# AmigoLab/SynthAnatomy

Measured on AMD Instinct MI355X. Metric: vqvae_train_volumes_per_sec, higher is better.
Workload: dtype bf16; 1 GPU; baseline_vqvae no_levels=4 no_channels=256 embedding_dim=32 num_embeddings=2048, 160x224x160 fp32 volumes, training step = fwd + MSE + bwd + EMA codebook update + Adam; batch_per_gpu=8, global_batch=8, parallelism=dp1

## Files before the change

### include/synthanatomy_hip.h

```cpp
#ifndef SYNTHANATOMY_HIP_H
#define SYNTHANATOMY_HIP_H
#include <stdint.h>

#ifdef __cplusplus
extern "C" {
#endif

#define SA_ABI_VERSION 5
enum { SA_F32 = 0, SA_BF16 = 1, SA_F16 = 2  };
enum { SA_ACT_NONE = 0, SA_ACT_RELU = 1, SA_ACT_LRELU = 2, SA_ACT_GELU = 3 };
enum { SA_MASK_NONE = 0, SA_MASK_POS = 1 , SA_MASK_LRELU = 2 ,
       SA_MASK_GELU = 3  };
enum { SA_EINVAL = -1, SA_EUNSUPPORTED = -2, SA_ENOGPU = -3, SA_ECOMM = -4  };
#define SA_MAX_TAPS 64

typedef struct sa_conv_geom {
    int32_t N, Dm, Hm, Wm;
    int32_t Di, Hi, Wi, Cin;
    int32_t Do, Ho, Wo, Cout;
    int32_t cin_valid, cout_valid;
    int32_t KT[3];
    int32_t in_mult[3], tap_step[3], in_off[3];
    int32_t out_mult[3], out_off[3];
    int32_t Kpad;
// ... 8 lines not shown
    int32_t act;
    int32_t mask_mode;
    int32_t add_before_act;
    int32_t out_dtype, add_dtype, mask_dtype;
    float slope;
    void *out_pre;
    void *out_lp;
} sa_epilogue;

int sa_abi_version(void);
const char *sa_last_error(void);
const char *sa_last_conv_kernel(void);
void sa_kernel_log_begin(void);
int sa_kernel_log_read(char *buf, int cap, int stop);

#define SA_DBG_NO_HALO           (1u << 0)
#define SA_DBG_NO_HALO256_FUSE   (1u << 2)
#define SA_DBG_NO_DMA            (1u << 3)
#define SA_DBG_NO_SMALL_TILES    (1u << 4)
#define SA_DBG_NO_FUSED_DB       (1u << 5)
#define SA_DBG_NO_WGRAD_HALO9    (1u << 6)
#define SA_DBG_IM2COL_DIRECT     (1u << 7)
#define SA_DBG_LOCAL_ATTN_EXACT  (1u << 9)
#define SA_DBG_HALO256_4W        (1u << 13)
#define SA_DBG_RESERVED_14       (1u << 14)
#define SA_DBG_DENSE_NARROW      (1u << 15)
#define SA_DBG_NO_KGROUPS        (1u << 17)
#define SA_DBG_RESERVED_19      (1u << 19)
#define SA_DBG_RESERVED_20      (1u << 20)
#define SA_DBG_NO_CELLS256       (1u << 21)
#define SA_DBG_NO_CLASS_LAUNCH    (1u << 22)
#define SA_DBG_NO_STRIP_TILES     (1u << 23)
#define SA_DBG_GENERIC_EPILOGUE   (1u << 24)
#define SA_DBG_FAVOR_SEQ_ALWAYS (1u << 18)
#define SA_DBG_DETERMINISTIC     (1u << 16)
#define SA_DBG_SCAN_EXACT_SHIFT  10
int sa_bench_mfma_bf16(float *scratch, int blocks, int iters, void *stream);
int sa_bench_mfma_bf16_ex(float *scratch, int blocks, int threads, int iters, int shape, void *stream);
uint32_t sa_get_debug_flags(void);
uint32_t sa_set_debug_flags(uint32_t flags);
int sa_epilogue_recipe(const sa_epilogue *ep, int dtype);

int sa_pack_weights(const float *w, void *wpk, int dtype, int rows, int red, int ntaps, const int32_t *tap_lut_host,
                    int64_t s_row, int64_t s_red, int rows_pad, int red_stride, int Kpad, void *stream);
typedef struct sa_pack_desc {
  const float *w;
  void *wpk;
  int32_t tap_lut[SA_MAX_TAPS];
  int64_t s_row, s_red;
  int32_t dtype, rows, red, ntaps, rows_pad, red_stride, Kpad, reserved;
} sa_pack_desc;
int sa_pack_weights_batch(const sa_pack_desc *table, const int32_t *block_first, int n, int total_blocks, void *stream);

int sa_conv_fprop(const sa_conv_geom *g, int dtype, const void *in, const void *wpk, void *out, const sa_epilogue *ep,
                  void *stream);
int sa_conv_fprop_classes(const sa_conv_geom *geoms, int n, int dtype, const void *in, const void *const *wpks, void *out, const sa_epilogue *ep,
                          void *stream);

int sa_resblock_fprop(const sa_conv_geom *g, int dtype, const void *x, const void *w3pk, const float *bias1, const void *w1pk, void *h_out,
                      void *y_out, const sa_epilogue *ep, void *stream);

int sa_conv_wgrad(const sa_conv_geom *g, int dtype, const void *in, const void *gout, float *dw, float *db, const int32_t *tap_lut_host,
                  int64_t s_row, int64_t s_red, void *workspace, int64_t workspace_bytes, void *stream);
int sa_conv1x1_backward(const sa_conv_geom *g, int dtype, const void *in, const void *gout, float *dw, float *db, int64_t s_row, int64_t s_red,
                        void *workspace, int64_t workspace_bytes, const void *dgrad_wpk, void *dx, void *stream);
int64_t sa_conv_wgrad_workspace_bytes(const sa_conv_geom *g, int dtype);

int sa_colsum(const void *g, int dtype, int64_t M, int C, int cstride, float *db, void *stream);

int sa_vq_assign(const float *rows, const float *codebook, int64_t M, int K, int D, int64_t *idx, float *zq_st, void *zq_lp,
                 float *counts, float *dw, float *sqerr, float *wnorm, void *stream);
int sa_vq_ema_update(float *N, float *embed_avg, float *codebook, const float *counts, const float *dw, int K, int D,
                     float decay, float eps, void *stream);
int sa_vq_restart_donors(const float *rows, int64_t M, int D, int64_t row_base, int64_t Mtot, int R, uint64_t seed, uint64_t step, float *donors,
                         void *stream);
int sa_vq_ema_update_restart(float *N, float *embed_avg, float *codebook, const float *counts, const float *dw, int K, int D, float decay, float eps,
                             int32_t *idle, int patience, const float *donors, int R, int32_t *info, void *stream);
int sa_vq_perplexity(const float *counts, int K, int64_t M, float *out, void *stream);
int sa_vq_backward(const float *rows, const float *codebook, const int64_t *idx, const void *g_zq, int g_dtype,
                   const float *g_loss, float beta, int64_t M, int D, void *dz, int dz_dtype, void *stream);
int sa_vq_embed(const float *codebook, const int64_t *idx, int64_t M, int K, int D, void *out, int out_dtype, void *stream);

int sa_cast_pad(const void *src, int src_dtype, int src_c, void *dst, int dst_dtype, int dst_stride, int64_t rows, void *stream);
int sa_subpixel_pool_fwd(const float *c, float *out, int N, int D, int H, int W, void *stream);
int sa_subpixel_pool_bwd(const float *g, void *dc, int dc_dtype, int N, int D, int H, int W, void *stream);
int sa_mse(const float *a, const float *b, int64_t n, float *loss_sum, float *grad, float gscale, void *stream);
int sa_baur_loss(const float *pred, const float *target, int64_t BC, int D, int H, int W, float gdl_factor, int reduction_sum, float gscale, float *sums3,
                 float *grad, float *ws, void *stream);
int64_t sa_baur_loss_workspace_bytes(int64_t BC, int D, int H, int W);
enum { SA_FOURIER_SPECTRAL = 0, SA_FOURIER_HARTLEY = 1, SA_FOURIER_WAVEGAN = 2 };
int sa_fourier_loss(int kind, const float *xp, const float *xy, int64_t B, int C, int D, int H, int W, int prioritise_hf, float factor, double *sums,
                    float *grad, void *ws, void *stream);
int64_t sa_fourier_loss_workspace_bytes(int64_t B, int C, int D, int H, int W);
int sa_ms_ssim(const float *x, const float *y, int B, int C, int D, int H, int W, const float *win, int win_size, int levels, const float *weights,
               float c1, float c2, float *out_b, float *level_means, void *ws, void *stream);
int64_t sa_ms_ssim_workspace_bytes(int B, int C, int D, int H, int W, int win_size, int levels);
enum { SA_AUG_IDENTITY = 0, SA_AUG_AFFINE = 1, SA_AUG_SIGNED_PERM = 2 };
enum { SA_AUG_GAMMA = 1, SA_AUG_SHIFT = 2, SA_AUG_NOISE = 4, SA_AUG_CLAMP = 8 };
typedef struct sa_augment_params {
// ... 262 lines not shown
```

### synthanatomy_amd/_ffi.py

```python
from __future__ import annotations

import ctypes
import os
from ctypes import POINTER, Structure, c_char_p, c_float, c_int, c_int32, c_int64, c_void_p

import torch

HERE = os.path.dirname(os.path.abspath(__file__))
LIB_PATH = os.environ.get("SA_HIP_LIB") or os.path.join(HERE, "libsynthanatomy_hip.so")

SA_F32, SA_BF16, SA_F16 = 0, 1, 2
ACT_NONE, ACT_RELU, ACT_LRELU, ACT_GELU = 0, 1, 2, 3
MASK_NONE, MASK_POS, MASK_LRELU, MASK_GELU = 0, 1, 2, 3
MAX_TAPS = 64


class ConvGeom(Structure):
    _fields_ = [
        ("N", c_int32), ("Dm", c_int32), ("Hm", c_int32), ("Wm", c_int32),
        ("Di", c_int32), ("Hi", c_int32), ("Wi", c_int32), ("Cin", c_int32),
        ("Do", c_int32), ("Ho", c_int32), ("Wo", c_int32), ("Cout", c_int32),
        ("cin_valid", c_int32), ("cout_valid", c_int32),
        ("KT", c_int32 * 3),
        ("in_mult", c_int32 * 3), ("tap_step", c_int32 * 3), ("in_off", c_int32 * 3),
# ... 67 lines not shown
    "sa_last_error": (c_char_p, []),
    "sa_last_conv_kernel": (c_char_p, []),
    "sa_kernel_log_begin": (None, []),
    "sa_kernel_log_read": (c_int, [ctypes.c_char_p, c_int, c_int]),
    "sa_bench_mfma_bf16": (c_int, [c_void_p, c_int, c_int, c_void_p]),
    "sa_bench_mfma_bf16_ex": (c_int, [c_void_p, c_int, c_int, c_int, c_int, c_void_p]),
    "sa_get_debug_flags": (ctypes.c_uint32, []),
    "sa_set_debug_flags": (ctypes.c_uint32, [ctypes.c_uint32]),
    "sa_epilogue_recipe": (c_int, [POINTER(Epilogue), c_int]),
    "sa_conv1_fwd": (c_int, [c_void_p, c_void_p, c_void_p, c_void_p, c_int, c_int, c_int, c_int, c_int, c_int, c_void_p]),
    "sa_conv1_fwd_f16": (c_int, [c_void_p, c_void_p, c_void_p, c_void_p, c_void_p, c_int, c_int, c_int, c_int, c_int, c_int, c_void_p]),
    "sa_conv1_wgrad": (c_int, [c_void_p, c_void_p, c_void_p, c_void_p, c_int, c_int, c_int, c_int, c_int, c_void_p]),
    "sa_convt1_fused_fwd": (c_int, [c_void_p, c_void_p, c_void_p, c_void_p, c_int, c_int, c_int, c_int, c_void_p]),
    "sa_convt1_backward": (c_int, [c_void_p, c_void_p, c_void_p, c_int, c_void_p, c_void_p, c_void_p, c_int, c_int, c_int, c_int, c_void_p]),
    "sa_favor_features_project_bwd": (c_int, [c_void_p, c_void_p, c_void_p, c_void_p, c_int, c_int, c_void_p, c_int, c_void_p, c_void_p, c_void_p, c_int64, c_int,
                                              c_int, c_int, c_void_p]),
    "sa_favor_project_features": (c_int, [c_void_p, c_int, c_int, c_void_p, c_void_p, c_void_p, c_int64, c_int, c_int, c_int, c_void_p]),
    "sa_favor_project": (c_int, [c_void_p, c_int, c_int, c_void_p, c_void_p, c_void_p, c_int64, c_int, c_int, c_int, c_void_p]),
    "sa_favor_project_bwd": (c_int, [c_void_p, c_void_p, c_void_p, c_void_p, c_int, c_int, c_int64, c_int, c_int, c_int, c_void_p]),
    "sa_favor_generalized_features_fwd": (c_int, [c_void_p, c_void_p, c_int64, c_int, c_int, c_void_p]),
    "sa_favor_generalized_features_bwd": (c_int, [c_void_p, c_void_p, c_void_p, c_int64, c_int, c_int, c_void_p]),
    "sa_favor_generalized_project_features": (c_int, [c_void_p, c_int, c_int, c_void_p, c_void_p, c_int64, c_int, c_int, c_int, c_int, c_int64, c_int64, c_void_p]),
    "sa_favor_generalized_project_bwd": (c_int, [c_void_p, c_void_p, c_void_p, c_void_p, c_int, c_int, c_int64, c_int, c_int, c_int, c_int, c_int64, c_int64,
                                                 c_void_p]),
    "sa_favor_generalized_step": (c_int, [c_void_p, c_int, c_int, c_void_p, c_int, c_int, c_void_p, c_int, c_int, c_void_p, c_int, c_int, c_int, c_int, c_int,
                                          c_void_p, c_void_p, c_void_p, c_void_p, c_void_p, c_int, c_int, c_void_p]),
    "sa_pack_weights_batch": (c_int, [c_void_p, c_void_p, c_int, c_int, c_void_p]),
    "sa_pack_weights": (c_int, [c_void_p, c_void_p, c_int, c_int, c_int, c_int, POINTER(c_int32), c_int64, c_int64, c_int, c_int, c_int, c_void_p]),
    "sa_conv_fprop": (c_int, [POINTER(ConvGeom), c_int, c_void_p, c_void_p, c_void_p, POINTER(Epilogue), c_void_p]),
    "sa_conv_fprop_classes": (c_int, [POINTER(ConvGeom), c_int, c_int, c_void_p, POINTER(c_void_p), c_void_p, POINTER(Epilogue), c_void_p]),
    "sa_resblock_fprop": (c_int, [POINTER(ConvGeom), c_int, c_void_p, c_void_p, c_void_p, c_void_p, c_void_p, c_void_p, POINTER(Epilogue), c_void_p]),
    "sa_conv_wgrad": (c_int, [POINTER(ConvGeom), c_int, c_void_p, c_void_p, c_void_p, c_void_p, POINTER(c_int32), c_int64, c_int64, c_void_p, c_int64, c_void_p]),
    "sa_conv_wgrad_workspace_bytes": (c_int64, [POINTER(ConvGeom), c_int]),
    "sa_conv1x1_backward": (c_int, [POINTER(ConvGeom), c_int, c_void_p, c_void_p, c_void_p, c_void_p, c_int64, c_int64, c_void_p, c_int64, c_void_p, c_void_p,
                                    c_void_p]),
    "sa_colsum": (c_int, [c_void_p, c_int, c_int64, c_int, c_int, c_void_p, c_void_p]),
    "sa_vq_assign": (c_int, [c_void_p, c_void_p, c_int64, c_int, c_int, c_void_p, c_void_p, c_void_p, c_void_p, c_void_p, c_void_p, c_void_p, c_void_p]),
    "sa_vq_ema_update": (c_int, [c_void_p, c_void_p, c_void_p, c_void_p, c_void_p, c_int, c_int, c_float, c_float, c_void_p]),
    "sa_vq_restart_donors": (c_int, [c_void_p, c_int64, c_int, c_int64, c_int64, c_int, ctypes.c_uint64, ctypes.c_uint64, c_void_p, c_void_p]),
    "sa_vq_ema_update_restart": (c_int, [c_void_p, c_void_p, c_void_p, c_void_p, c_void_p, c_int, c_int, c_float, c_float, c_void_p, c_int, c_void_p, c_int,
                                         c_void_p, c_void_p]),
    "sa_vq_perplexity": (c_int,[c_void_p, c_int, c_int64, c_void_p, c_void_p]),
    "sa_vq_backward": (c_int, [c_void_p, c_void_p, c_void_p, c_void_p, c_int, c_void_p, c_float, c_int64, c_int, c_void_p, c_int, c_void_p]),
    "sa_vq_embed": (c_int, [c_void_p, c_void_p, c_int64, c_int, c_int, c_void_p, c_int, c_void_p]),
    "sa_cast_pad": (c_int, [c_void_p, c_int, c_int, c_void_p, c_int, c_int, c_int64, c_void_p]),
    "sa_mse": (c_int, [c_void_p, c_void_p, c_int64, c_void_p, c_void_p, c_float, c_void_p]),
    "sa_mse_det": (c_int, [c_void_p, c_void_p, c_int64, c_void_p, c_void_p, c_float, c_void_p, c_void_p]),
    "sa_baur_loss": (c_int, [c_void_p, c_void_p, c_int64, c_int, c_int, c_int, c_float, c_int, c_float, c_void_p, c_void_p, c_void_p, c_void_p]),
    "sa_baur_loss_workspace_bytes": (c_int64, [c_int64, c_int, c_int, c_int]),
    "sa_fourier_loss": (c_int, [c_int, c_void_p, c_void_p, c_int64, c_int, c_int, c_int, c_int, c_int, c_float, c_void_p, c_void_p, c_void_p, c_void_p]),
    "sa_fourier_loss_workspace_bytes": (c_int64, [c_int64, c_int, c_int, c_int, c_int]),
    "sa_ms_ssim": (c_int, [c_void_p, c_void_p, c_int, c_int, c_int, c_int, c_int, c_void_p, c_int, c_int, c_void_p, c_float, c_float, c_void_p, c_void_p,
                           c_void_p, c_void_p]),
    "sa_ms_ssim_workspace_bytes": (c_int64, [c_int, c_int, c_int, c_int, c_int, c_int, c_int]),
    "sa_augment": (c_int, [c_void_p, c_void_p, c_int, c_int, c_int, c_int, c_int, c_int, c_int, c_void_p, ctypes.c_uint64, c_void_p, c_void_p]),
    "sa_augment_workspace_bytes": (c_int64, [c_int]),
    "sa_volume_ingest": (c_int, [c_void_p, c_int64, c_void_p, c_void_p, c_void_p, c_void_p]),
    "sa_volume_ingest_workspace_bytes": (c_int64, []),
    "sa_volume_egress": (c_int, [c_void_p, c_void_p, c_int64, c_void_p, c_void_p, c_void_p]),
    "sa_volume_egress_workspace_bytes": (c_int64, []),
    "sa_anomaly_map": (c_int, [c_void_p, c_void_p, c_void_p, c_void_p, c_void_p, POINTER(AnomalyParams), c_void_p, c_void_p, c_void_p]),
    "sa_anomaly_map_workspace_bytes": (c_int64, [POINTER(AnomalyParams)]),
    "sa_anomaly_map_ensemble": (c_int, [c_void_p, c_void_p, c_int64, c_void_p, c_int64, c_void_p, c_void_p, POINTER(AnomalyParams), c_int, c_void_p,
                                        c_void_p, c_void_p]),
    "sa_components": (c_int, [c_void_p, c_void_p, c_void_p, POINTER(ComponentsParams), c_void_p, c_void_p, c_void_p]),
    "sa_components_workspace_bytes": (c_int64, [POINTER(ComponentsParams)]),
# ... 183 lines not shown
```

### synthanatomy_amd/csrc/conv_wgrad.hip

```cpp
#include <stdio.h>
#include <stdlib.h>

#include "sa_common.h"

namespace sa {

struct WgradArgs {
    const void* in;
    const void* gout;
    float* dw;
    sa_conv_geom g;
    FastDiv dW, dH, dD, dTw, dThw, dCin;
    int32_t lut[SA_MAX_TAPS];
    int64_t s_row, s_red;
    uint32_t M, ntaps, ktot;
    uint32_t chunks_per_split, nchunks;
    uint32_t nkt, ntiles;
    uint32_t in_bytes, g_bytes;
    float* ws;
    float* db;
    const void* dg_wpk;
    void* dg_out;
    uint32_t HQ, WP, nsteps, steps_per_split, halo;
    FastDiv dWP, dHQ;
};

template <typename T> struct WG;
template <> struct WG<bf16_t> { static constexpr int MK = 64; };
template <> struct WG<float> { static constexpr int MK = 16; };

__device__ __forceinline__ uint32_t roff(uint32_t m, uint32_t c) { return m * 256u + ((((c >> 4) ^ (m & 7u)) << 5) | ((c & 15u) << 1)); }

typedef short v4s_t __attribute__((ext_vector_type(4)));
__device__ __forceinline__ v4s_t lds_tr16(const unsigned char* p) {
    return __builtin_amdgcn_ds_read_tr16_b64_v4i16((__attribute__((address_space(3))) v4s_t*)(p));
}

__device__ __forceinline__ void dma16_hidden(__amdgpu_buffer_rsrc_t rsrc, uint32_t lds_addr, uint32_t voff) {
    asm volatile("s_mov_b32 m0, %0\n\ts_nop 0\n\tbuffer_load_dwordx4 %1, %2, 0 offen lds" : : "s"(lds_addr), "v"(voff), "s"(rsrc) : "memory", "m0");
}
__device__ __forceinline__ void dma_wait() { asm volatile("s_waitcnt vmcnt(0)" ::: "memory"); }
__device__ __forceinline__ uint32_t lds_address(const void* p) { return (uint32_t)(uintptr_t)(__attribute__((address_space(3))) const void*)p; }

template <int ROWS, int NGROUPS>
__device__ __forceinline__ void tile_colsum(const unsigned char* pg, uint32_t tid, float& s0, float& s1) {
    const uint32_t cp = tid & 63u, rg = tid >> 6;
#pragma unroll
    for (int m = 0; m < ROWS / NGROUPS + (ROWS % NGROUPS ? 1 : 0); ++m) {
        const uint32_t row = rg + (uint32_t)m * NGROUPS;
        if (ROWS % NGROUPS == 0 || row < (uint32_t)ROWS) {
            const uint32_t v = *(const uint32_t*)(pg + roff(row, 2u * cp));
            s0 += __uint_as_float(v << 16);
            s1 += __uint_as_float(v & 0xffff0000u);
        }
    }
}
// ... 548 lines not shown
        for (int ks = 0; ks < PHS / 2; ++ks) {
            short8_t xf[4], gf[4];
            const uint32_t xr0 = (uint32_t)(2 * ks) * 18u + tw + trow, xr1 = xr0 + 18u;
#pragma unroll
            for (int i = 0; i < 4; ++i) {
                const v4s_t lo = lds_tr16(px + roff(xr0, wm * 64 + i * 16 + tcol));
                const v4s_t hi = lds_tr16(px + roff(xr1, wm * 64 + i * 16 + tcol));
                xf[i] = __builtin_shufflevector(lo, hi, 0, 1, 2, 3, 4, 5, 6, 7);
            }
#pragma unroll
            for (int j = 0; j < 4; ++j) {
                const v4s_t lo = lds_tr16(pg + roff(ks * 32 + trow, wn * 64 + j * 16 + tcol));
                const v4s_t hi = lds_tr16(pg + roff(ks * 32 + 16 + trow, wn * 64 + j * 16 + tcol));
                gf[j] = __builtin_shufflevector(lo, hi, 0, 1, 2, 3, 4, 5, 6, 7);
            }
#pragma unroll
            for (int i = 0; i < 4; ++i)
#pragma unroll
                for (int j = 0; j < 4; ++j) acc[i][j] = __builtin_amdgcn_mfma_f32_16x16x32_bf16(xf[i], gf[j], acc[i][j], 0, 0, 0);
        }
        __syncthreads();
    }
    if (do_db) colsum_finish<12>((float*)smem, tid, bs0, bs1, a.db, ct * 128u, (uint32_t)g.cout_valid);
    const uint32_t tile = (td * 3u + th) * 3u + tw + a.nkt * ct;
    float* wt = a.ws + ((size_t)split * a.ntiles + tile) * (128 * 128);
#pragma unroll
    for (int i = 0; i < 4; ++i)
#pragma unroll
        for (int j = 0; j < 4; ++j) *(float4_t*)(wt + (wn * 64 + j * 16 + frow) * 128 + wm * 64 + i * 16 + fq * 4) = acc[i][j];
#endif
}

__device__ __forceinline__ uint32_t roff128(uint32_t m, uint32_t c) { return m * 128u + ((((c >> 4) ^ ((m >> 1) & 3u)) << 5) | ((c & 15u) << 1)); }

template <int NW>
__global__ __launch_bounds__(NW * 64) void conv_wgrad_halo9_kernel(const WgradArgs a) {
#if defined(__HIP_DEVICE_COMPILE__)
    constexpr int NJ = 32 / NW;
    constexpr int XP = 23, GP = 32, NP = XP + GP, PPW = (NP + NW - 1) / NW;
    constexpr int XT = XP * 1024, GT = GP * 1024, STAGE = XT + GT;
    extern __shared__ __attribute__((aligned(16))) unsigned char smem[];
    const sa_conv_geom& g = a.g;
    const uint32_t tid = threadIdx.x, lane = tid & 63u;
    const uint32_t wave = __builtin_amdgcn_readfirstlane(tid >> 6);
    const uint32_t fi = wave & 3u, wn = wave >> 2;
    const uint32_t nct = a.ntiles / a.nkt;
    const uint32_t xcd = blockIdx.x & 7u, seq = blockIdx.x >> 3;
    const uint32_t per_split = 6u * nct;
    const uint32_t nsplit = (a.nsteps + a.steps_per_split - 1) / a.steps_per_split;
    const uint32_t spx = (nsplit + 7u) >> 3;
    const uint32_t sl = seq / per_split, rem = seq - sl * per_split;
    const uint32_t split = xcd * spx + sl;
    if (sl >= spx || split >= nsplit) return;
    const uint32_t tdc = rem % 6u, ct = rem / 6u;
    const uint32_t td = tdc >> 1, cih = tdc & 1u;
    const uint32_t step0 = split * a.steps_per_split;
    uint32_t step1 = step0 + a.steps_per_split;
    if (step1 > a.nsteps) step1 = a.nsteps;

    float4_t acc[9][NJ];
#pragma unroll
    for (int t = 0; t < 9; ++t)
#pragma unroll
        for (int j = 0; j < NJ; ++j) acc[t][j] = (float4_t){0.f, 0.f, 0.f, 0.f};

    __amdgpu_buffer_rsrc_t rX = __builtin_amdgcn_make_buffer_rsrc((void*)a.in, 0, (int)a.in_bytes, 0x00020000);
// ... 18 lines not shown
            p_h[i] = (int32_t)(r >> 4);
            p_w[i] = (int32_t)(r & 15u);
            p_off[i] = (uint32_t)((p_h[i] * g.Wo + p_w[i]) * (g.Cout * 2)) + ct * 256u + vec * 16u;
        }
    }
    auto issue = [&](uint32_t step, uint32_t buf) __attribute__((always_inline)) {
        const uint32_t ps = smem_addr + buf * STAGE;
        uint32_t q1 = fdiv(step, a.dWP);
        const uint32_t wp = step - q1 * a.WP;
        uint32_t q2 = fdiv(q1, a.dHQ);
        const uint32_t hq = q1 - q2 * a.HQ;
        const uint32_t n = fdiv(q2, a.dD);
        const uint32_t d = q2 - n * (uint32_t)g.Dm;
        const int32_t h0 = (int32_t)hq * 8, w0 = (int32_t)wp * 16;
        const int32_t id = (int32_t)d + g.in_off[0] + (int32_t)td;
        const bool dok = (uint32_t)id < (uint32_t)g.Di;
        const uint32_t xbase = (uint32_t)((((int32_t)n * g.Di + id) * g.Hi + h0) * g.Wi + w0) * (uint32_t)(g.Cin * 2);
        const uint32_t gbase = (uint32_t)((((int32_t)n * g.Do + (int32_t)d) * g.Ho + h0) * g.Wo + w0) * (uint32_t)(g.Cout * 2);
#pragma unroll
        for (int i = 0; i < PPW; ++i) {
            const uint32_t q = wave + (uint32_t)NW * i;
            if (q >= (uint32_t)NP) break;
            const int32_t hh = h0 + p_h[i], ww = w0 + p_w[i];
            if (q < (uint32_t)XP) {
                const bool ok = dok && (uint32_t)hh < (uint32_t)g.Hi && (uint32_t)ww < (uint32_t)g.Wi;
                dma16_hidden(rX, ps + q * 1024, ok ? xbase + p_off[i] : 0xfffffff0u);
            } else {
                const bool ok = (uint32_t)hh < (uint32_t)g.Ho && (uint32_t)ww < (uint32_t)g.Wo;
                dma16_hidden(rG, ps + XT + (q - (uint32_t)XP) * 1024, ok ? gbase + p_off[i] : 0xfffffff0u);
            }
        }
    };

    issue(step0, 0);
    dma_wait();
    __syncthreads();
    const uint32_t frow = lane & 15u, fq = lane >> 4;
    const uint32_t trow = fq * 4u + (frow >> 2), tcol = (frow & 3u) * 4u;
    const bool do_db = a.db != nullptr && tdc == 0u;
    float bs0 = 0.f, bs1 = 0.f;
    uint32_t xa[9][2];
#pragma unroll
    for (int t = 0; t < 9; ++t) {
        const uint32_t xr0 = (uint32_t)(t / 3) * 18u + (uint32_t)(t % 3) + trow;
        xa[t][0] = roff128(xr0, fi * 16 + tcol);
        xa[t][1] = roff128(xr0 + 18u, fi * 16 + tcol);
    }
    uint32_t ga[NJ];
#pragma unroll
    for (int j = 0; j < NJ; ++j) ga[j] = roff(trow, wn * (16 * NJ) + j * 16 + tcol);
    for (uint32_t st = step0; st < step1; ++st) {
        const uint32_t buf = (st - step0) & 1u;
        if (st + 1 < step1) issue(st + 1, buf ^ 1u);
        const unsigned char* px = smem + buf * STAGE;
        const unsigned char* pg = px + XT;
        if (do_db) tile_colsum<128, NW>(pg, tid, bs0, bs1);
#pragma unroll 1
        for (uint32_t ks = 0; ks < 4; ++ks) {
            short8_t gf[NJ];
            const unsigned char* pgk = pg + ks * 8192u;
            const unsigned char* pxk = px + ks * 4608u;
            const uint32_t kx = (ks & 1u) * 64u;
#pragma unroll
            for (int j = 0; j < NJ; ++j) {
                const v4s_t lo = lds_tr16(pgk + ga[j]);
                const v4s_t hi = lds_tr16(pgk + ga[j] + 4096);
                gf[j] = __builtin_shufflevector(lo, hi, 0, 1, 2, 3, 4, 5, 6, 7);
            }
#pragma unroll
            for (int t = 0; t < 9; ++t) {
                const v4s_t lo = lds_tr16(pxk + (xa[t][0] ^ kx));
                const v4s_t hi = lds_tr16(pxk + (xa[t][1] ^ kx));
                const short8_t xf = __builtin_shufflevector(lo, hi, 0, 1, 2, 3, 4, 5, 6, 7);
#pragma unroll
                for (int j = 0; j < NJ; ++j) acc[t][j] = __builtin_amdgcn_mfma_f32_16x16x32_bf16(xf, gf[j], acc[t][j], 0, 0, 0);
            }
        }
        dma_wait();
        __syncthreads();
    }
    if (do_db) colsum_finish<NW>((float*)smem, tid, bs0, bs1, a.db, ct * 128u, (uint32_t)g.cout_valid);
#pragma unroll
    for (int t = 0; t < 9; ++t) {
        float* wt = a.ws + ((size_t)split * a.ntiles + (td * 9u + t) + a.nkt * ct) * (128 * 128);
#pragma unroll
        for (int j = 0; j < NJ; ++j) *(float4_t*)(wt + (wn * (16 * NJ) + j * 16 + frow) * 128 + cih * 64 + fi * 16 + fq * 4) = acc[t][j];
    }
#endif
}

__global__ __launch_bounds__(256) void wgrad_reduce_kernel(const WgradArgs a, uint32_t splits) {
    const uint32_t e4 = blockIdx.x * blockDim.x + threadIdx.x;
    if (e4 >= a.ntiles * 4096u) return;
    const uint32_t e = e4 * 4u;
    const uint32_t tile = e >> 14, co_l = (e >> 7) & 127u, k_l = e & 127u;
    const uint32_t kt = tile % a.nkt, ct = tile / a.nkt;
    const uint32_t kidx = kt * 128u + k_l, co = ct * 128u + co_l;
    if (kidx >= a.ktot || co >= (uint32_t)a.g.cout_valid) return;
    float4_t s = (float4_t){0.f, 0.f, 0.f, 0.f};
    const float* p = a.ws + e;
    const size_t stride = (size_t)a.ntiles * 16384u;
    uint32_t sp = 0;
    for (; sp + 8 <= splits; sp += 8) {
        float4_t v[8];
#pragma unroll
        for (int u = 0; u < 8; ++u) v[u] = __builtin_nontemporal_load((const float4_t*)(p + (size_t)(sp + u) * stride));
#pragma unroll
        for (int u = 0; u < 8; ++u) s += v[u];
    }
    for (; sp < splits; ++sp) s += *(const float4_t*)(p + (size_t)sp * stride);
#pragma unroll
    for (int r = 0; r < 4; ++r) {
        const uint32_t kk = kidx + r;
        if (kk >= a.ktot) break;
        const uint32_t tap = fdiv(kk, a.dCin);
        const uint32_t c = kk - tap * a.g.Cin;
        if (c >= (uint32_t)a.g.cin_valid) continue;
        a.dw[co * a.s_row + (int64_t)c * a.s_red + a.lut[tap]] += s[r];
    }
}

__global__ __launch_bounds__(1024) void wgrad_reduce_wide_kernel(const WgradArgs a, uint32_t splits) {
// ... 101 lines not shown
    const int64_t M = (int64_t)g->N * g->Dm * g->Hm * g->Wm;
    if (M <= 0 || M >= (1ll << 31)) return SA_EINVAL;
    a.g = *g;
    a.dW = make_fastdiv(g->Wm);
    a.dH = make_fastdiv(g->Hm);
    a.dD = make_fastdiv(g->Dm);
    a.dTw = make_fastdiv(g->KT[2]);
    a.dThw = make_fastdiv(g->KT[1] * g->KT[2]);
    a.dCin = make_fastdiv(g->Cin);
    a.M = (uint32_t)M;
    a.ntaps = ntaps;
    a.ktot = ntaps * g->Cin;
    const int mk = dtype == SA_F32 ? 16 : 64;
    a.nchunks = (uint32_t)((M + mk - 1) / mk);
    a.nkt = (a.ktot + 127) / 128;
    const uint32_t nct = ((uint32_t)g->cout_valid + 127) / 128;
    a.ntiles = a.nkt * nct;
    const int target_rows = g_tunables.wgrad_rows;
    const uint32_t want_cps = (uint32_t)(target_rows / mk) ? (uint32_t)(target_rows / mk) : 1u;
    splits = (a.nchunks + want_cps - 1) / want_cps;
    const uint32_t env_blocks = (uint32_t)g_tunables.wgrad_min_blocks;
    const uint32_t min_blocks = env_blocks ? env_blocks : ((ntaps == 1 && a.nchunks <= 1024u) ? 512u : 1024u);
    const uint32_t min_splits = (min_blocks + a.ntiles - 1) / a.ntiles;
    if (splits < min_splits) splits = min_splits;
    const uint32_t cap = (uint32_t)((2ull << 30) / ((uint64_t)a.ntiles * 65536ull));
    if (splits > cap && cap >= 1) splits = cap;
    const uint32_t min_chunks = dtype == SA_F32 ? 16 : 4;
    uint32_t max_splits = (a.nchunks + min_chunks - 1) / min_chunks;
    if (splits > max_splits) splits = max_splits;
    if (splits < 1) splits = 1;
    a.chunks_per_split = (a.nchunks + splits - 1) / splits;
    splits = (a.nchunks + a.chunks_per_split - 1) / a.chunks_per_split;
    a.halo = 0;
    {
        bool ok = dtype == SA_BF16 && g->Cin == 128 && g->cin_valid == 128 && g->Cout % 128 == 0 && !dbg(SA_DBG_NO_HALO) && !dbg(SA_DBG_NO_DMA);
        for (int d = 0; d < 3 && ok; ++d)
            ok = g->KT[d] == 3 && g->in_mult[d] == 1 && g->tap_step[d] == 1 && g->in_off[d] == -1 && g->out_mult[d] == 1 && g->out_off[d] == 0;
        ok = ok && g->Dm == g->Do && g->Hm == g->Ho && g->Wm == g->Wo && g->Di == g->Do && g->Hi == g->Ho && g->Wi == g->Wo;
        const uint64_t ib = (uint64_t)g->N * g->Di * g->Hi * g->Wi * g->Cin * 2, gb = (uint64_t)g->N * g->Do * g->Ho * g->Wo * g->Cout * 2;
        ok = ok && ib < 0xffffff00ull - (1u << 20) && gb < 0xffffff00ull - (1u << 20);
        if (ok) {
            const bool nine = !dbg(SA_DBG_NO_WGRAD_HALO9);
            const uint32_t phs = nine ? 8u : 4u;
            const uint32_t hq = (uint32_t)(g->Ho + phs - 1) / phs, wp = (uint32_t)(g->Wo + 15) / 16;
            const double eff = (double)g->Ho * g->Wo / ((double)hq * phs * wp * 16);
            const uint64_t nsteps = (uint64_t)g->N * g->Dm * hq * wp;
            if (eff >= 0.8 && nsteps >= 512) {
                a.halo = nine ? 9u : 4u;
                a.HQ = hq;
                a.WP = wp;
                a.nsteps = (uint32_t)nsteps;
                a.dWP = make_fastdiv(wp);
                a.dHQ = make_fastdiv(hq);
                const int want = g_tunables.wgrad_halo_splits ? g_tunables.wgrad_halo_splits : (nine ? 128 : 256);
                uint32_t sp = (uint32_t)want;
                if (sp > a.nsteps / 16) sp = a.nsteps / 16;
                if (sp < 1) sp = 1;
                a.steps_per_split = (a.nsteps + sp - 1) / sp;
                splits = (a.nsteps + a.steps_per_split - 1) / a.steps_per_split;
            }
        }
    }
    return 0;
}
}

extern "C" int64_t sa_conv_wgrad_workspace_bytes(const sa_conv_geom* g, int dtype) {
    using namespace sa;
    if (!g) return SA_EINVAL;
    WgradArgs a;
    uint32_t splits;
    const int rc = plan_wgrad(g, dtype, a, splits);
    if (rc) return rc;
    return (int64_t)splits * a.ntiles * 128 * 128 * 4;
}

extern "C" int sa_colsum(const void* gp, int dtype, int64_t M, int C, int cstride, float* db, void* stream);

static int conv_wgrad_impl(const sa_conv_geom* g, int dtype, const void* in, const void* gout, float* dw, float* db, const int32_t* tap_lut_host,
                           int64_t s_row, int64_t s_red, void* workspace, int64_t workspace_bytes, const void* dg_wpk, void* dg_out, void* stream) {
    using namespace sa;
    if (!g || !in || !gout || !dw) return SA_EINVAL;
    WgradArgs a;
    uint32_t splits;
    const int rc = plan_wgrad(g, dtype, a, splits);
    if (rc) return rc;
    a.in = in;
    a.gout = gout;
    a.dw = dw;
    const int ntaps = a.ntaps;
    for (int t = 0; t < SA_MAX_TAPS; ++t) a.lut[t] = tap_lut_host ? (t < ntaps ? tap_lut_host[t] : 0) : t;
    a.s_row = s_row;
    a.s_red = s_red;
    const int64_t need = (int64_t)splits * a.ntiles * 128 * 128 * 4;
    a.ws = (workspace && workspace_bytes >= need) ? (float*)workspace : nullptr;
    if (workspace && !a.ws) return SA_EINVAL;
    a.db = nullptr;
    const size_t lds = dtype == SA_F32 ? 4 * 8192 : 4 * 16384;
    const uint32_t splits8 = (splits + 7u) & ~7u;
    dim3 grid(a.ntiles * splits8);
    hipStream_t st = (hipStream_t)stream;
    {
        const int sz = dtype == SA_F32 ? 4 : 2;
        const uint64_t ib = (uint64_t)g->N * g->Di * g->Hi * g->Wi * g->Cin * sz, gb = (uint64_t)g->N * g->Do * g->Ho * g->Wo * g->Cout * sz;
        const bool fits = ib < 0xffffff00ull && gb < 0xffffff00ull && !dbg(SA_DBG_NO_DMA);
        a.in_bytes = fits ? (uint32_t)ib : 0u;
        a.g_bytes = fits ? (uint32_t)gb : 0u;
// ... 92 lines not shown
```

### synthanatomy_amd/csrc/elementwise.hip

```cpp
#include "sa_common.h"

#include <cstring>
#include <mutex>
#include <string>

namespace sa {

thread_local hipError_t g_last_error = hipSuccess;
thread_local char g_last_conv_kernel[128] = "";
std::atomic<bool> g_kernel_log_on{false};
static std::mutex g_kernel_log_mu;
static std::string* g_kernel_log = nullptr;
void note_kernel_slow(const char* name) {
    std::lock_guard<std::mutex> lk(g_kernel_log_mu);
    if (!g_kernel_log) g_kernel_log = new std::string();
    std::string key(name);
    if (key.size() > 2 && key.front() == '(' && key.back() == ')') key = key.substr(1, key.size() - 2);
    key.push_back('\n');
    if (g_kernel_log->rfind(key, 0) == 0 || g_kernel_log->find("\n" + key) != std::string::npos) return;
    g_kernel_log->append(key);
}

static uint32_t flags_from_env() {
    auto on = [](const char* n) { return getenv(n) != nullptr; };
    auto num = [](const char* n, int dflt) { const char* e = getenv(n); return e ? atoi(e) : dflt; };
    uint32_t f = 0;
    if (on("SA_NO_HALO")) f |= SA_DBG_NO_HALO;
    if (on("SA_NO_HALO256_FUSE")) f |= SA_DBG_NO_HALO256_FUSE;
    if (on("SA_NO_DMA")) f |= SA_DBG_NO_DMA;
    if (on("SA_NO_SMALL_TILES")) f |= SA_DBG_NO_SMALL_TILES;
    if (on("SA_NO_FUSED_DB")) f |= SA_DBG_NO_FUSED_DB;
    if (getenv("SA_WGRAD_HALO9") && num("SA_WGRAD_HALO9", 1) == 0) f |= SA_DBG_NO_WGRAD_HALO9;
    if (on("SA_IM2COL_DIRECT")) f |= SA_DBG_IM2COL_DIRECT;
    if (on("SA_HALO256_4W")) f |= SA_DBG_HALO256_4W;
    if (on("SA_DENSE_NARROW")) f |= SA_DBG_DENSE_NARROW;
    if (on("SA_DETERMINISTIC")) f |= SA_DBG_DETERMINISTIC;
    if (on("SA_NO_KGROUPS")) f |= SA_DBG_NO_KGROUPS;
    if (on("SA_FAVOR_SEQ_ALWAYS")) f |= SA_DBG_FAVOR_SEQ_ALWAYS;
    if (on("SA_NO_CELLS256")) f |= SA_DBG_NO_CELLS256;
    if (on("SA_NO_CLASS_LAUNCH")) f |= SA_DBG_NO_CLASS_LAUNCH;
    if (on("SA_GENERIC_EPILOGUE")) f |= SA_DBG_GENERIC_EPILOGUE;
    if (num("SA_LOCAL_ATTN_EXACT", 0) == 1) f |= SA_DBG_LOCAL_ATTN_EXACT;
    f |= ((uint32_t)num("SA_SCAN_EXACT", 0) & 7u) << SA_DBG_SCAN_EXACT_SHIFT;
    return f;
}
static Tunables tunables_from_env() {
    auto num = [](const char* n, int dflt) { const char* e = getenv(n); return e ? atoi(e) : dflt; };
    return Tunables{num("SA_WGRAD_ROWS", 10240), num("SA_WGRAD_MIN_BLOCKS", 0), num("SA_WGRAD_HALO_SPLITS", 0), (uint32_t)num("SA_PP_DBG", 0)};
}
std::atomic<uint32_t> g_debug_flags{flags_from_env()};
const Tunables g_tunables = tunables_from_env();

struct PackArgs {
    const float* w;
    void* wpk;
    int32_t lut[SA_MAX_TAPS];
    int64_t s_row, s_red;
    int32_t dtype, rows, red, ntaps, rows_pad, red_stride, Kpad;
};

__global__ void pack_weights_kernel(const PackArgs a) {
    const int64_t total = (int64_t)a.rows_pad * a.Kpad;
    for (int64_t e = (int64_t)blockIdx.x * blockDim.x + threadIdx.x; e < total; e += (int64_t)gridDim.x * blockDim.x) {
        const int r = (int)(e / a.Kpad);
        const int k = (int)(e - (int64_t)r * a.Kpad);
        const int t = k / a.red_stride;
        const int c = k - t * a.red_stride;
        float v = 0.f;
        if (r < a.rows && t < a.ntaps && c < a.red) v = a.w[r * a.s_row + c * a.s_red + a.lut[t]];
        store_from_f32(a.wpk, a.dtype, e, v);
    }
}

__global__ __launch_bounds__(256) void pack_weights_batch_kernel(const sa_pack_desc* __restrict__ table, const int32_t* __restrict__ block_first, int n) {
// ... 411 lines not shown
```

### synthanatomy_amd/debug.py

```python
from __future__ import annotations

import contextlib
import os

LIB_FLAGS = dict(no_halo=1 << 0, no_halo256_fuse=1 << 2, no_dma=1 << 3, no_small_tiles=1 << 4, no_fused_db=1 << 5,
                 no_wgrad_halo9=1 << 6, im2col_direct=1 << 7, local_attn_exact=1 << 9, halo256_4w=1 << 13, dense_narrow=1 << 15, deterministic=1 << 16, no_kgroups=1 << 17, favor_seq_always=1 << 18, no_cells256=1 << 21, no_class_launch=1 << 22, no_strip_tiles=1 << 23, generic_epilogue=1 << 24)
SCAN_EXACT_SHIFT = 10

_HOST_ENV = dict(no_fused_res="SA_NO_FUSED_RES", no_fused_1x1_bwd="SA_NO_FUSED_1X1_BWD", no_fused_qkv="SA_NO_FUSED_QKV", no_fused_favor="SA_NO_FUSED_FAVOR",
                 no_convt1_fused_bwd="SA_NO_CONVT1_FUSED_BWD", no_convt1_fused_fwd="SA_NO_CONVT1_FUSED_FWD", no_side_wgrad="SA_NO_SIDE_WGRAD", no_side_wgrad_vqvae="SA_NO_SIDE_WGRAD_VQVAE",
                 ddp_single_rank="SA_DDP_SINGLE_RANK",
                 no_f16_forward="SA_NO_F16_FORWARD",
                 no_sample_step="SA_NO_SAMPLE_STEP",
                 opt_in_backward="SA_OPT_IN_BACKWARD",
                 share_device="SA_SHARE_DEVICE",
                 no_proj_bf16="SA_NO_PROJ_BF16",
                 keep_ipc_mode="SA_KEEP_IPC_MODE")
_host = {k: os.environ.get(v) is not None for k, v in _HOST_ENV.items()}


def host(name: str) -> bool:
    return _host[name]


def deterministic() -> bool:
    from . import _ffi
    return bool(_ffi.lib().sa_get_debug_flags() & LIB_FLAGS["deterministic"])


def set_deterministic(on: bool = True):
    from . import _ffi
    lib = _ffi.lib()
    f = lib.sa_get_debug_flags()
    lib.sa_set_debug_flags((f | LIB_FLAGS["deterministic"]) if on else (f & ~LIB_FLAGS["deterministic"]))


@contextlib.contextmanager
def override(**kw):
    from . import _ffi
# ... 21 lines not shown
```

Before: 73.33 volumes/s.

## Restructure halo9 wgrad main loop with incremental walk, precomputed masks and staggered DMA

Result: faster. 74.58 volumes/s (median of 6 runs) (+1.7%).

```diff
diff --git a/include/synthanatomy_hip.h b/include/synthanatomy_hip.h
--- a/include/synthanatomy_hip.h
+++ b/include/synthanatomy_hip.h
@@ -64,6 +64,8 @@
 #define SA_DBG_NO_CLASS_LAUNCH    (1u << 22)
 #define SA_DBG_NO_STRIP_TILES     (1u << 23)
 #define SA_DBG_GENERIC_EPILOGUE   (1u << 24)
+#define SA_DBG_WGRAD9_LOCKSTEP    (1u << 25)
+#define SA_DBG_WGRAD9_FORCE       (1u << 26)
 #define SA_DBG_FAVOR_SEQ_ALWAYS (1u << 18)
 #define SA_DBG_DETERMINISTIC     (1u << 16)
 #define SA_DBG_SCAN_EXACT_SHIFT  10
@@ -97,6 +99,7 @@
 int sa_conv1x1_backward(const sa_conv_geom *g, int dtype, const void *in, const void *gout, float *dw, float *db, int64_t s_row, int64_t s_red,
                         void *workspace, int64_t workspace_bytes, const void *dgrad_wpk, void *dx, void *stream);
 int64_t sa_conv_wgrad_workspace_bytes(const sa_conv_geom *g, int dtype);
+int sa_wgrad9_step_walk(uint32_t WP, uint32_t HQ, uint32_t Dm, uint32_t step0, uint32_t count, uint32_t *out);
 
 int sa_colsum(const void *g, int dtype, int64_t M, int C, int cstride, float *db, void *stream);
 
diff --git a/synthanatomy_amd/_ffi.py b/synthanatomy_amd/_ffi.py
--- a/synthanatomy_amd/_ffi.py
+++ b/synthanatomy_amd/_ffi.py
@@ -123,6 +123,7 @@
     "sa_resblock_fprop": (c_int, [POINTER(ConvGeom), c_int, c_void_p, c_void_p, c_void_p, c_void_p, c_void_p, c_void_p, POINTER(Epilogue), c_void_p]),
     "sa_conv_wgrad": (c_int, [POINTER(ConvGeom), c_int, c_void_p, c_void_p, c_void_p, c_void_p, POINTER(c_int32), c_int64, c_int64, c_void_p, c_int64, c_void_p]),
     "sa_conv_wgrad_workspace_bytes": (c_int64, [POINTER(ConvGeom), c_int]),
+    "sa_wgrad9_step_walk": (c_int, [ctypes.c_uint32, ctypes.c_uint32, ctypes.c_uint32, ctypes.c_uint32, ctypes.c_uint32, POINTER(ctypes.c_uint32)]),
     "sa_conv1x1_backward": (c_int, [POINTER(ConvGeom), c_int, c_void_p, c_void_p, c_void_p, c_void_p, c_int64, c_int64, c_void_p, c_int64, c_void_p, c_void_p,
                                     c_void_p]),
     "sa_colsum": (c_int, [c_void_p, c_int, c_int64, c_int, c_int, c_void_p, c_void_p]),
diff --git a/synthanatomy_amd/csrc/conv_wgrad.hip b/synthanatomy_amd/csrc/conv_wgrad.hip
--- a/synthanatomy_amd/csrc/conv_wgrad.hip
+++ b/synthanatomy_amd/csrc/conv_wgrad.hip
@@ -1,5 +1,7 @@
 #include <stdio.h>
 #include <stdlib.h>
+
+#include <type_traits>
 
 #include "sa_common.h"
 
@@ -22,6 +24,7 @@
     const void* dg_wpk;
     void* dg_out;
     uint32_t HQ, WP, nsteps, steps_per_split, halo;
+    uint32_t wg9_lockstep;
     FastDiv dWP, dHQ;
 };
 
@@ -636,6 +639,56 @@
 }
 
 __device__ __forceinline__ uint32_t roff128(uint32_t m, uint32_t c) { return m * 128u + ((((c >> 4) ^ ((m >> 1) & 3u)) << 5) | ((c & 15u) << 1)); }
+
+struct Wgrad9Walk {
+    uint32_t wp, hq, d, n;
+};
+__host__ __device__ inline Wgrad9Walk wgrad9_walk_at(uint32_t step, uint32_t WP, uint32_t HQ, uint32_t Dm) {
+    Wgrad9Walk w;
+    const uint32_t q1 = step / WP, q2 = q1 / HQ;
+    w.wp = step - q1 * WP;
+    w.hq = q1 - q2 * HQ;
+    w.n = q2 / Dm;
+    w.d = q2 - w.n * Dm;
+    return w;
+}
+__host__ __device__ inline void wgrad9_walk_next(Wgrad9Walk& w, uint32_t WP, uint32_t HQ, uint32_t Dm) {
+    if (++w.wp != WP) return;
+    w.wp = 0;
+    if (++w.hq != HQ) return;
+    w.hq = 0;
+    if (++w.d != Dm) return;
+    w.d = 0;
+    ++w.n;
+}
+
+__device__ __forceinline__ v4s_t lds_tr16_at(uint32_t addr) {
+    return __builtin_amdgcn_ds_read_tr16_b64_v4i16((__attribute__((address_space(3))) v4s_t*)(size_t)addr);
+}
+
+#ifdef SA_TIMING
+#define SA_WG9_TROWS 4096
+__device__ unsigned long long g_wg9_timing[SA_WG9_TROWS * 16];
+#define WG9_TNOW(v)                                                                                  \
+    do {                                                                                             \
+        __builtin_amdgcn_sched_barrier(0);                                                           \
+        asm volatile("s_memtime %0\n\ts_waitcnt lgkmcnt(0)" : "=s"(v)::"memory");                     \
+        __builtin_amdgcn_sched_barrier(0);                                                           \
+    } while (0)
+#define WG9_T(slot)                          \
+    do {                                     \
+        unsigned long long t_now_;           \
+        WG9_TNOW(t_now_);                    \
+        wg9_ts[slot] += t_now_ - wg9_tprev;  \
+        wg9_tprev = t_now_;                  \
+    } while (0)
+#else
+#define WG9_T(slot)
+#endif
+
+#ifndef SA_WG9_STAGGER
+#define SA_WG9_STAGGER 1
+#endif
 
 template <int NW>
 __global__ __launch_bounds__(NW * 64) void conv_wgrad_halo9_kernel(const WgradArgs a) {
@@ -720,9 +773,10 @@
         }
     };
 
-    issue(step0, 0);
-    dma_wait();
-    __syncthreads();
+#ifdef SA_TIMING
+    unsigned long long wg9_ts[8] = {0, 0, 0, 0, 0, 0, 0, 0}, wg9_tprev;
+    WG9_TNOW(wg9_tprev);
+#endif
     const uint32_t frow = lane & 15u, fq = lane >> 4;
     const uint32_t trow = fq * 4u + (frow >> 2), tcol = (frow & 3u) * 4u;
     const bool do_db = a.db != nullptr && tdc == 0u;
@@ -737,45 +791,192 @@
     uint32_t ga[NJ];
 #pragma unroll
     for (int j = 0; j < NJ; ++j) ga[j] = roff(trow, wn * (16 * NJ) + j * 16 + tcol);
-    for (uint32_t st = step0; st < step1; ++st) {
-        const uint32_t buf = (st - step0) & 1u;
-        if (st + 1 < step1) issue(st + 1, buf ^ 1u);
-        const unsigned char* px = smem + buf * STAGE;
-        const unsigned char* pg = px + XT;
-        if (do_db) tile_colsum<128, NW>(pg, tid, bs0, bs1);
-#pragma unroll 1
-        for (uint32_t ks = 0; ks < 4; ++ks) {
-            short8_t gf[NJ];
-            const unsigned char* pgk = pg + ks * 8192u;
-            const unsigned char* pxk = px + ks * 4608u;
-            const uint32_t kx = (ks & 1u) * 64u;
-#pragma unroll
-            for (int j = 0; j < NJ; ++j) {
-                const v4s_t lo = lds_tr16(pgk + ga[j]);
-                const v4s_t hi = lds_tr16(pgk + ga[j] + 4096);
-                gf[j] = __builtin_shufflevector(lo, hi, 0, 1, 2, 3, 4, 5, 6, 7);
-            }
-#pragma unroll
-            for (int t = 0; t < 9; ++t) {
-                const v4s_t lo = lds_tr16(pxk + (xa[t][0] ^ kx));
-                const v4s_t hi = lds_tr16(pxk + (xa[t][1] ^ kx));
-                const short8_t xf = __builtin_shufflevector(lo, hi, 0, 1, 2, 3, 4, 5, 6, 7);
-#pragma unroll
-                for (int j = 0; j < NJ; ++j) acc[t][j] = __builtin_amdgcn_mfma_f32_16x16x32_bf16(xf, gf[j], acc[t][j], 0, 0, 0);
-            }
-        }
+    const bool lockstep = NW != 8 || a.wg9_lockstep != 0u || (smem_addr & 127u) != 0u;
+    if (lockstep) {
+        issue(step0, 0);
         dma_wait();
         __syncthreads();
+        WG9_T(6);
+        for (uint32_t st = step0; st < step1; ++st) {
+            const uint32_t buf = (st - step0) & 1u;
+            if (st + 1 < step1) issue(st + 1, buf ^ 1u);
+            WG9_T(0);
+            const unsigned char* px = smem + buf * STAGE;
+            const unsigned char* pg = px + XT;
+            if (do_db) tile_colsum<128, NW>(pg, tid, bs0, bs1);
+            WG9_T(1);
+#pragma unroll 1
+            for (uint32_t ks = 0; ks < 4; ++ks) {
+                short8_t gf[NJ];
+                const unsigned char* pgk = pg + ks * 8192u;
+                const unsigned char* pxk = px + ks * 4608u;
+                const uint32_t kx = (ks & 1u) * 64u;
+#pragma unroll
+                for (int j = 0; j < NJ; ++j) {
+                    const v4s_t lo = lds_tr16(pgk + ga[j]);
+                    const v4s_t hi = lds_tr16(pgk + ga[j] + 4096);
+                    gf[j] = __builtin_shufflevector(lo, hi, 0, 1, 2, 3, 4, 5, 6, 7);
+                }
+#pragma unroll
+                for (int t = 0; t < 9; ++t) {
+                    const v4s_t lo = lds_tr16(pxk + (xa[t][0] ^ kx));
+                    const v4s_t hi = lds_tr16(pxk + (xa[t][1] ^ kx));
+                    const short8_t xf = __builtin_shufflevector(lo, hi, 0, 1, 2, 3, 4, 5, 6, 7);
+                    if (t == 0) WG9_T(2);
+#pragma unroll
+                    for (int j = 0; j < NJ; ++j) acc[t][j] = __builtin_amdgcn_mfma_f32_16x16x32_bf16(xf, gf[j], acc[t][j], 0, 0, 0);
+                }
+                WG9_T(3);
+            }
+            dma_wait();
+            WG9_T(4);
+            __syncthreads();
+            WG9_T(5);
+        }
+    } else {
+        __builtin_assume(wave < (uint32_t)NW);
+        constexpr int NPM = (PPW + 4) / 5;
+        uint32_t pm[NPM];
+#pragma unroll
+        for (int i = 0; i < NPM; ++i) pm[i] = 0u;
+        const int32_t hl = (int32_t)(a.HQ - 1u) * 8, wl = (int32_t)(a.WP - 1u) * 16;
+#pragma unroll
+        for (int i = 0; i < PPW; ++i) {
+            const uint32_t q = wave + (uint32_t)NW * i;
+            uint32_t f;
+            if (q < (uint32_t)XP)
+                f = (p_h[i] < 0 ? 1u : 0u) | (hl + p_h[i] >= g.Hi ? 2u : 0u) | (p_w[i] < 0 ? 4u : 0u) | (wl + p_w[i] >= g.Wi ? 8u : 0u) | (p_h[i] < -1 ? 16u : 0u) | 32u;
+            else
+                f = (hl + p_h[i] >= g.Ho ? 2u : 0u) | (wl + p_w[i] >= g.Wo ? 8u : 0u);
+            pm[i / 5] |= f << (6 * (i % 5));
+        }
+        auto issue2 = [&](const Wgrad9Walk& w, uint32_t buf) __attribute__((always_inline)) {
+            const uint32_t ps = smem_addr + buf * STAGE;
+            const int32_t h0 = (int32_t)w.hq * 8, w0 = (int32_t)w.wp * 16;
+            const int32_t id = (int32_t)w.d + g.in_off[0] + (int32_t)td;
+            const bool dok = (uint32_t)id < (uint32_t)g.Di;
+            const uint32_t xbase = (uint32_t)((((int32_t)w.n * g.Di + id) * g.Hi + h0) * g.Wi + w0) * (uint32_t)(g.Cin * 2);
+            const uint32_t gbase = (uint32_t)((((int32_t)w.n * g.Do + (int32_t)w.d) * g.Ho + h0) * g.Wo + w0) * (uint32_t)(g.Cout * 2);
+            const uint32_t em = (w.hq == 0u ? 1u : 0u) | (w.hq + 1u == a.HQ ? 2u : 0u) | (w.wp == 0u ? 4u : 0u) | (w.wp + 1u == a.WP ? 8u : 0u) | 16u | (dok ? 0u : 32u);
+#pragma unroll
+            for (int i = 0; i < PPW; ++i) {
+                const uint32_t q = wave + (uint32_t)NW * i;
+                if (q >= (uint32_t)NP) break;
+                const bool ok = (pm[i / 5] & (em << (6 * (i % 5)))) == 0u;
+                if (q < (uint32_t)XP) dma16_hidden(rX, ps + q * 1024, ok ? xbase + p_off[i] : 0xfffffff0u);
+                else dma16_hidden(rG, ps + XT + (q - (uint32_t)XP) * 1024, ok ? gbase + p_off[i] : 0xfffffff0u);
+            }
+        };
+        Wgrad9Walk walk;
+        {
+            const uint32_t q1 = fdiv(step0, a.dWP), q2 = fdiv(q1, a.dHQ);
+            walk.wp = step0 - q1 * a.WP;
+            walk.hq = q1 - q2 * a.HQ;
+            walk.n = fdiv(q2, a.dD);
+            walk.d = q2 - walk.n * (uint32_t)g.Dm;
+        }
+        issue2(walk, 0);
+        uint32_t xr[9][2], gr[NJ];
+#pragma unroll
+        for (int t = 0; t < 9; ++t) {
+            xr[t][0] = smem_addr + xa[t][0];
+            xr[t][1] = smem_addr + xa[t][1];
+        }
+#pragma unroll
+        for (int j = 0; j < NJ; ++j) gr[j] = smem_addr + (uint32_t)XT + ga[j];
+        auto kstep = [&](auto ksc) __attribute__((always_inline)) {
+            constexpr uint32_t KS = decltype(ksc)::value;
+            short8_t gf[NJ];
+#pragma unroll
+            for (int j = 0; j < NJ; ++j) {
+                const v4s_t lo = lds_tr16_at(gr[j] + KS * 8192u);
+                const v4s_t hi = lds_tr16_at(gr[j] + KS * 8192u + 4096u);
+                gf[j] = __builtin_shufflevector(lo, hi, 0, 1, 2, 3, 4, 5, 6, 7);
+            }
+#pragma unroll
+            for (int t = 0; t < 9; ++t) {
+                const v4s_t lo = lds_tr16_at((xr[t][0] ^ ((KS & 1u) * 64u)) + KS * 4608u);
+                const v4s_t hi = lds_tr16_at((xr[t][1] ^ ((KS & 1u) * 64u)) + KS * 4608u);
+                const short8_t xf = __builtin_shufflevector(lo, hi, 0, 1, 2, 3, 4, 5, 6, 7);
+                if (t == 0) WG9_T(2);
+#pragma unroll
+                for (int j = 0; j < NJ; ++j) acc[t][j] = __builtin_amdgcn_mfma_f32_16x16x32_bf16(xf, gf[j], acc[t][j], 0, 0, 0);
+            }
+            WG9_T(3);
+            __builtin_amdgcn_sched_barrier(0);
+        };
+        dma_wait();
+        __syncthreads();
+        WG9_T(6);
+        const bool late = SA_WG9_STAGGER && wave >= (uint32_t)NW / 2u;
+        for (uint32_t st = step0; st < step1; ++st) {
+            const uint32_t buf = (st - step0) & 1u;
+            const bool more = st + 1 < step1;
+            if (more) wgrad9_walk_next(walk, a.WP, a.HQ, (uint32_t)g.Dm);
+            if (more && !late) issue2(walk, buf ^ 1u);
+            WG9_T(0);
+            if (do_db) tile_colsum<128, NW>(smem + buf * STAGE + XT, tid, bs0, bs1);
+            WG9_T(1);
+            kstep(std::integral_constant<uint32_t, 0>{});
+            if (more && late) issue2(walk, buf ^ 1u);
+            WG9_T(0);
+            kstep(std::integral_constant<uint32_t, 1>{});
+            kstep(std::integral_constant<uint32_t, 2>{});
+            kstep(std::integral_constant<uint32_t, 3>{});
+            const uint32_t flip = buf ? 0u - (uint32_t)STAGE : (uint32_t)STAGE;
+#pragma unroll
+            for (int t = 0; t < 9; ++t) {
+                xr[t][0] += flip;
+                xr[t][1] += flip;
+            }
+#pragma unroll
+            for (int j = 0; j < NJ; ++j) gr[j] += flip;
+            dma_wait();
+            WG9_T(4);
+            __syncthreads();
+            WG9_T(5);
+        }
     }
     if (do_db) colsum_finish<NW>((float*)smem, tid, bs0, bs1, a.db, ct * 128u, (uint32_t)g.cout_valid);
+    WG9_T(1);
 #pragma unroll
     for (int t = 0; t < 9; ++t) {
         float* wt = a.ws + ((size_t)split * a.ntiles + (td * 9u + t) + a.nkt * ct) * (128 * 128);
 #pragma unroll
         for (int j = 0; j < NJ; ++j) *(float4_t*)(wt + (wn * (16 * NJ) + j * 16 + frow) * 128 + cih * 64 + fi * 16 + fq * 4) = acc[t][j];
     }
+#ifdef SA_TIMING
+    asm volatile("s_waitcnt vmcnt(0)" ::: "memory");
+    WG9_T(7);
+    {
+        unsigned long long* tl = (unsigned long long*)smem;
+        __syncthreads();
+        if ((wave == 0u || wave == (uint32_t)NW / 2u) && lane < 8u) {
+            unsigned long long v = 0;
+#pragma unroll
+            for (int k = 0; k < 8; ++k)
+                if (lane == (uint32_t)k) v = wg9_ts[k];
+            tl[(wave ? 8u : 0u) + lane] = v;
+        }
+        __syncthreads();
+        if (tid < 16u && blockIdx.x < (uint32_t)SA_WG9_TROWS) g_wg9_timing[blockIdx.x * 16u + tid] += tl[tid];
+    }
 #endif
-}
+#endif
+}
+
+#ifdef SA_TIMING
+}
+extern "C" int sa_debug_timing_wgrad9(unsigned long long* out, int reset) {
+    if (out) hipMemcpyFromSymbol(out, HIP_SYMBOL(sa::g_wg9_timing), sizeof(unsigned long long) * SA_WG9_TROWS * 16);
+    if (reset) {
+        void* p = nullptr;
+        if (hipGetSymbolAddress(&p, HIP_SYMBOL(sa::g_wg9_timing)) == hipSuccess) hipMemset(p, 0, sizeof(unsigned long long) * SA_WG9_TROWS * 16);
+    }
+    return 0;
+}
+namespace sa {
+#endif
 
 __global__ __launch_bounds__(256) void wgrad_reduce_kernel(const WgradArgs a, uint32_t splits) {
     const uint32_t e4 = blockIdx.x * blockDim.x + threadIdx.x;
@@ -943,6 +1144,7 @@
     a.chunks_per_split = (a.nchunks + splits - 1) / splits;
     splits = (a.nchunks + a.chunks_per_split - 1) / a.chunks_per_split;
     a.halo = 0;
+    a.wg9_lockstep = dbg(SA_DBG_WGRAD9_LOCKSTEP) ? 1u : 0u;
     {
         bool ok = dtype == SA_BF16 && g->Cin == 128 && g->cin_valid == 128 && g->Cout % 128 == 0 && !dbg(SA_DBG_NO_HALO) && !dbg(SA_DBG_NO_DMA);
         for (int d = 0; d < 3 && ok; ++d)
@@ -956,7 +1158,8 @@
             const uint32_t hq = (uint32_t)(g->Ho + phs - 1) / phs, wp = (uint32_t)(g->Wo + 15) / 16;
             const double eff = (double)g->Ho * g->Wo / ((double)hq * phs * wp * 16);
             const uint64_t nsteps = (uint64_t)g->N * g->Dm * hq * wp;
-            if (eff >= 0.8 && nsteps >= 512) {
+            const bool force9 = nine && dbg(SA_DBG_WGRAD9_FORCE) && nsteps < (1ull << 31);
+            if ((eff >= 0.8 && nsteps >= 512) || force9) {
                 a.halo = nine ? 9u : 4u;
                 a.HQ = hq;
                 a.WP = wp;
@@ -966,6 +1169,10 @@
                 const int want = g_tunables.wgrad_halo_splits ? g_tunables.wgrad_halo_splits : (nine ? 128 : 256);
                 uint32_t sp = (uint32_t)want;
                 if (sp > a.nsteps / 16) sp = a.nsteps / 16;
+                if (force9 && !(eff >= 0.8 && nsteps >= 512)) {
+                    sp = a.nsteps >= 6 ? (a.nsteps + 2) / 3 : 2;
+                    if (sp > (uint32_t)want) sp = (uint32_t)want;
+                }
                 if (sp < 1) sp = 1;
                 a.steps_per_split = (a.nsteps + sp - 1) / sp;
                 splits = (a.nsteps + a.steps_per_split - 1) / a.steps_per_split;
@@ -984,6 +1191,16 @@
     const int rc = plan_wgrad(g, dtype, a, splits);
     if (rc) return rc;
     return (int64_t)splits * a.ntiles * 128 * 128 * 4;
+}
+
+extern "C" int sa_wgrad9_step_walk(uint32_t WP, uint32_t HQ, uint32_t Dm, uint32_t step0, uint32_t count, uint32_t* out) {
+    if (!WP || !HQ || !Dm || !out) return SA_EINVAL;
+    sa::Wgrad9Walk w = sa::wgrad9_walk_at(step0, WP, HQ, Dm);
+    for (uint32_t i = 0; i < count; ++i) {
+        out[4 * i + 0] = w.wp, out[4 * i + 1] = w.hq, out[4 * i + 2] = w.d, out[4 * i + 3] = w.n;
+        sa::wgrad9_walk_next(w, WP, HQ, Dm);
+    }
+    return 0;
 }
 
 extern "C" int sa_colsum(const void* gp, int dtype, int64_t M, int C, int cstride, float* db, void* stream);
diff --git a/synthanatomy_amd/csrc/elementwise.hip b/synthanatomy_amd/csrc/elementwise.hip
--- a/synthanatomy_amd/csrc/elementwise.hip
+++ b/synthanatomy_amd/csrc/elementwise.hip
@@ -40,6 +40,8 @@
     if (on("SA_NO_CELLS256")) f |= SA_DBG_NO_CELLS256;
     if (on("SA_NO_CLASS_LAUNCH")) f |= SA_DBG_NO_CLASS_LAUNCH;
     if (on("SA_GENERIC_EPILOGUE")) f |= SA_DBG_GENERIC_EPILOGUE;
+    if (on("SA_WGRAD9_LOCKSTEP")) f |= SA_DBG_WGRAD9_LOCKSTEP;
+    if (on("SA_WGRAD9_FORCE")) f |= SA_DBG_WGRAD9_FORCE;
     if (num("SA_LOCAL_ATTN_EXACT", 0) == 1) f |= SA_DBG_LOCAL_ATTN_EXACT;
     f |= ((uint32_t)num("SA_SCAN_EXACT", 0) & 7u) << SA_DBG_SCAN_EXACT_SHIFT;
     return f;
diff --git a/synthanatomy_amd/debug.py b/synthanatomy_amd/debug.py
--- a/synthanatomy_amd/debug.py
+++ b/synthanatomy_amd/debug.py
@@ -4,7 +4,7 @@
 import os
 
 LIB_FLAGS = dict(no_halo=1 << 0, no_halo256_fuse=1 << 2, no_dma=1 << 3, no_small_tiles=1 << 4, no_fused_db=1 << 5,
-                 no_wgrad_halo9=1 << 6, im2col_direct=1 << 7, local_attn_exact=1 << 9, halo256_4w=1 << 13, dense_narrow=1 << 15, deterministic=1 << 16, no_kgroups=1 << 17, favor_seq_always=1 << 18, no_cells256=1 << 21, no_class_launch=1 << 22, no_strip_tiles=1 << 23, generic_epilogue=1 << 24)
+                 no_wgrad_halo9=1 << 6, im2col_direct=1 << 7, local_attn_exact=1 << 9, halo256_4w=1 << 13, dense_narrow=1 << 15, deterministic=1 << 16, no_kgroups=1 << 17, favor_seq_always=1 << 18, no_cells256=1 << 21, no_class_launch=1 << 22, no_strip_tiles=1 << 23, generic_epilogue=1 << 24, wgrad9_lockstep=1 << 25, wgrad9_force=1 << 26)
 SCAN_EXACT_SHIFT = 10
 
 _HOST_ENV = dict(no_fused_res="SA_NO_FUSED_RES", no_fused_1x1_bwd="SA_NO_FUSED_1X1_BWD", no_fused_qkv="SA_NO_FUSED_QKV", no_fused_favor="SA_NO_FUSED_FAVOR",
```
